# CagriCatik/RRT-MPC

Hardware: AMD Instinct MI355X
Metric: MPC QP solves/s (horizon=20, batch=4096) @1/2/4/8 GPU; rel-err vs OSQP (higher is better)
Workload: dtype f64

## Files before the change

### rrt-mpc_amd/csrc/mpcqp_common.h

```cpp
#pragma once
#include <hip/hip_runtime.h>

#include <chrono>
#include <cmath>
#include <cstdint>
#include <cstdio>
#include <cstring>
#include <functional>
#include <mutex>
#include <new>
#include <string>
#include <type_traits>
#include <utility>

#include "../../include/mpcqp.h"

namespace {

constexpr int kWave = 64;
constexpr double kPi = 3.141592653589793;
constexpr double kTwoPi = 6.283185307179586;
constexpr double kMinScaling = 1e-4;
constexpr double kMaxScaling = 1e4;
constexpr double kRhoMin = 1e-6;
// ... 79 lines not shown
  double off = row >= 1 ? t0 : 0.0;
  if (row >= 2) off = fmax(off, t1);
  if (row >= 3) off = fmax(off, t2);
  return fmax(v, off);
}
__device__ __forceinline__ double rscan_max(double v, int lane) {
  v = fmax(v, dpp<kRowShl1>(v));
  v = fmax(v, dpp<kRowShl2>(v));
  v = fmax(v, dpp<kRowShl4>(v));
  v = fmax(v, dpp<kRowShl8>(v));
  const double t1 = readlane(v, 16), t2 = readlane(v, 32), t3 = readlane(v, 48);
  const int row = lane >> 4;
  double off = row <= 2 ? t3 : 0.0;
  if (row <= 1) off = fmax(off, t2);
  if (row <= 0) off = fmax(off, t1);
  return fmax(v, off);
}
__device__ __forceinline__ double max_nc(double a, double b) {
  double r;
  asm("v_max_f64 %0, %1, %2" : "=v"(r) : "v"(a), "v"(b));
  return r;
}
__device__ __forceinline__ double min_nc(double a, double b) {
  double r;
  asm("v_min_f64 %0, %1, %2" : "=v"(r) : "v"(a), "v"(b));
  return r;
}
__device__ __forceinline__ double wave_sum(double v) { return readlane(scan_add(v, 0), 63); }
__device__ __forceinline__ void wave_sum2(double& a, double& b) {
  a += dpp<kRowShr1>(a);
  b += dpp<kRowShr1>(b);
  a += dpp<kRowShr2>(a);
  b += dpp<kRowShr2>(b);
  a += dpp<kRowShr4>(a);
  b += dpp<kRowShr4>(b);
  a += dpp<kRowShr8>(a);
  b += dpp<kRowShr8>(b);
  a += dpp_rows<kRowBcast15, 0xa>(a);
  b += dpp_rows<kRowBcast15, 0xa>(b);
  a += dpp_rows<kRowBcast31, 0xc>(a);
  b += dpp_rows<kRowBcast31, 0xc>(b);
  a = readlane(a, 63);
  b = readlane(b, 63);
}
__device__ __forceinline__ double wave_max(double v) {
  v = max_nc(v, dpp<kRowShr1>(v));
  v = max_nc(v, dpp<kRowShr2>(v));
  v = max_nc(v, dpp<kRowShr4>(v));
  v = max_nc(v, dpp<kRowShr8>(v));
  v = max_nc(v, dpp_rows<kRowBcast15, 0xa>(v));
  v = max_nc(v, dpp_rows<kRowBcast31, 0xc>(v));
  return readlane(v, 63);
}
#define MPCQP_MAX4_STEP(MOVE)                                             \
  {                                                                       \
    const double ta = MOVE(a), tb = MOVE(b), tc = MOVE(c), td = MOVE(d); \
    a = max_nc(a, ta);                                                    \
    b = max_nc(b, tb);                                                    \
    c = max_nc(c, tc);                                                    \
    d = max_nc(d, td);                                                    \
  }
__device__ __forceinline__ void half_max4_steps(double& a, double& b, double& c, double& d) {
  MPCQP_MAX4_STEP(dpp<kRowShr1>)
  MPCQP_MAX4_STEP(dpp<kRowShr2>)
  MPCQP_MAX4_STEP(dpp<kRowShr4>)
  MPCQP_MAX4_STEP(dpp<kRowShr8>)
  MPCQP_MAX4_STEP((dpp_rows<kRowBcast15, 0xa>))
}
__device__ __forceinline__ void wave_max4(double& a, double& b, double& c, double& d) {
  half_max4_steps(a, b, c, d);
  MPCQP_MAX4_STEP((dpp_rows<kRowBcast31, 0xc>))
  a = readlane(a, 63);
  b = readlane(b, 63);
  c = readlane(c, 63);
  d = readlane(d, 63);
}
#undef MPCQP_MAX4_STEP
__device__ __forceinline__ double shr2(double v) { return dpp<kWaveShr1>(dpp<kWaveShr1>(v)); }
__device__ __forceinline__ double shl2(double v) { return dpp<kWaveShl1>(dpp<kWaveShl1>(v)); }
__device__ __forceinline__ double shr4(double v) { return shr2(shr2(v)); }
__device__ __forceinline__ double shl4(double v) { return shl2(shl2(v)); }
__device__ __forceinline__ bool wave_any(bool b) { return __ballot(b) != 0ull; }

template <int NW>
__device__ __forceinline__ void bcast(double v, double w[4]) {
  const int lo = __double2loint(v), hi = __double2hiint(v);
  const auto l16 = __builtin_amdgcn_permlane16_swap(lo, lo, false, false);
  const auto h16 = __builtin_amdgcn_permlane16_swap(hi, hi, false, false);
  const auto la = __builtin_amdgcn_permlane32_swap(l16[0], l16[0], false, false);
  const auto ha = __builtin_amdgcn_permlane32_swap(h16[0], h16[0], false, false);
  w[0] = __hiloint2double(ha[0], la[0]);
  if constexpr (NW > 1) {
    const auto lb = __builtin_amdgcn_permlane32_swap(l16[1], l16[1], false, false);
    const auto hb = __builtin_amdgcn_permlane32_swap(h16[1], h16[1], false, false);
    w[1] = __hiloint2double(hb[0], lb[0]);
    if constexpr (NW > 3) w[3] = __hiloint2double(hb[1], lb[1]);
  }
  if constexpr (NW > 2) w[2] = __hiloint2double(ha[1], la[1]);
  if constexpr (NW == 1) asm volatile("s_nop 1" : "+v"(w[0]));
  if constexpr (NW == 2) asm volatile("s_nop 1" : "+v"(w[0]), "+v"(w[1]));
  if constexpr (NW == 3) asm volatile("s_nop 1" : "+v"(w[0]), "+v"(w[1]), "+v"(w[2]));
  if constexpr (NW == 4) asm volatile("s_nop 1" : "+v"(w[0]), "+v"(w[1]), "+v"(w[2]), "+v"(w[3]));
}
template <int NW>
__device__ __forceinline__ void bcast_rows01(double v, double w[4]) {
  static_assert(NW <= 2, "two 16-lane rows");
  if constexpr (NW == 1) {
    w[0] = v;
    asm volatile("s_nop 1" : "+v"(w[0]));
  } else {
    const int lo = __double2loint(v), hi = __double2hiint(v);
    const auto l16 = __builtin_amdgcn_permlane16_swap(lo, lo, false, false);
    const auto h16 = __builtin_amdgcn_permlane16_swap(hi, hi, false, false);
    w[0] = __hiloint2double(h16[0], l16[0]);
    w[1] = __hiloint2double(h16[1], l16[1]);
    asm volatile("s_nop 1" : "+v"(w[0]), "+v"(w[1]));
  }
}
template <int L>
__device__ __forceinline__ void fmac_bc(double& acc, double w, double m) {
  asm("v_fmac_f64_dpp %0, %1, %2 row_newbcast:%3 row_mask:0xf bank_mask:0xf" : "+v"(acc) : "v"(w), "v"(m), "i"(L));
}
template <bool Pair>
struct Lanes;

template <>
struct Lanes<false> {
  static constexpr int kLanes = kWave;
  template <int NW>
  __device__ __forceinline__ static void vbcast(double v, double w[4]) {
    if constexpr (NW <= 2)
      bcast_rows01<NW>(v, w);
    else
      bcast<NW>(v, w);
  }
  template <int K>
  __device__ __forceinline__ static double read(double v) { return readlane(v, K); }
  __device__ __forceinline__ static double readv(double v, int l) { return readlane(v, l); }
  __device__ __forceinline__ static int uniform(int l) { return __builtin_amdgcn_readfirstlane(l); }
  __device__ __forceinline__ static double sum(double v) { return wave_sum(v); }
  __device__ __forceinline__ static void sum2(double& a, double& b) { wave_sum2(a, b); }
  __device__ __forceinline__ static double max(double v) { return wave_max(v); }
  __device__ __forceinline__ static void max4(double& a, double& b, double& c, double& d) { wave_max4(a, b, c, d); }
  __device__ __forceinline__ static bool any(bool b) { return wave_any(b); }
  __device__ __forceinline__ static uint64_t ballot(bool b) { return __ballot(b); }
  __device__ __forceinline__ static double shr2(double v) { return ::shr2(v); }
  __device__ __forceinline__ static double shl2(double v) { return ::shl2(v); }
  __device__ __forceinline__ static double shr4(double v) { return ::shr4(v); }
  __device__ __forceinline__ static double shl4(double v) { return ::shl4(v); }
  __device__ __forceinline__ static double shr1(double v) { return dpp<kWaveShr1>(v); }
  __device__ __forceinline__ static double shl1(double v) { return dpp<kWaveShl1>(v); }
  __device__ __forceinline__ static double scan(double v, int lane) { return scan_add(v, lane); }
  __device__ __forceinline__ static double shfl(double v, int src) { return __shfl(v, src, kWave); }
};

template <int L>
__device__ __forceinline__ double row_bc(double v) {
  const int lo = __builtin_amdgcn_update_dpp(0, __double2loint(v), 0x150 + L, 0xf, 0xf, false);
  const int hi = __builtin_amdgcn_update_dpp(0, __double2hiint(v), 0x150 + L, 0xf, 0xf, false);
  return __hiloint2double(hi, lo);
}

template <>
struct Lanes<true> {
  static constexpr int kLanes = 32;
  __device__ __forceinline__ static int hl() { return (int)threadIdx.x & 31; }
  __device__ __forceinline__ static double pin(double v) {
    asm volatile("" : "+v"(v));
    return v;
  }
  template <int NW>
  __device__ __forceinline__ static void vbcast(double v, double w[4]) {
    static_assert(NW <= 2, "a half holds 32 lanes");
    bcast_rows01<2>(v, w);
  }
  template <int K>
  __device__ __forceinline__ static double read(double v) {
    double w[4];
    bcast_rows01<2>(v, w);
    return pin(row_bc<K % 16>(w[K / 16]));
  }
  __device__ __forceinline__ static double readv(double v, int l) { return pin(__shfl(v, l, 32)); }
  __device__ __forceinline__ static int uniform(int l) { return l; }
  __device__ __forceinline__ static double scan(double v, int lane) {
    (void)lane;
    v += dpp<kRowShr1>(v);
    v += dpp<kRowShr2>(v);
    v += dpp<kRowShr4>(v);
    v += dpp<kRowShr8>(v);
    v += dpp_rows<kRowBcast15, 0xa>(v);
    return pin(v);
  }
  __device__ __forceinline__ static double sum(double v) { return read<31>(scan(v, 0)); }
  __device__ __forceinline__ static void sum2(double& a, double& b) {
    a = sum(a);
    b = sum(b);
  }
  __device__ __forceinline__ static double max(double v) {
    v = max_nc(v, dpp<kRowShr1>(v));
    v = max_nc(v, dpp<kRowShr2>(v));
    v = max_nc(v, dpp<kRowShr4>(v));
    v = max_nc(v, dpp<kRowShr8>(v));
    v = max_nc(v, dpp_rows<kRowBcast15, 0xa>(v));
    return read<31>(v);
  }
  __device__ __forceinline__ static void max4(double& a, double& b, double& c, double& d) {
    half_max4_steps(a, b, c, d);
    a = read<31>(a);
    b = read<31>(b);
    c = read<31>(c);
    d = read<31>(d);
  }
  __device__ __forceinline__ static uint64_t ballot(bool b) {
    const uint64_t m = __ballot(b);
    return (threadIdx.x & 32) ? (m >> 32) : (m & 0xffffffffull);
  }
  __device__ __forceinline__ static bool any(bool b) { return ballot(b) != 0ull; }
  __device__ __forceinline__ static double shr2(double v) {
    const double d = pin(::shr2(v));
    return hl() >= 2 ? d : 0.0;
  }
  __device__ __forceinline__ static double shl2(double v) {
    const double d = pin(::shl2(v));
    return hl() < 30 ? d : 0.0;
  }
  __device__ __forceinline__ static double shr4(double v) { return shr2(shr2(v)); }
  __device__ __forceinline__ static double shl4(double v) { return shl2(shl2(v)); }
  __device__ __forceinline__ static double shr1(double v) {
    const double d = pin(dpp<kWaveShr1>(v));
    return hl() >= 1 ? d : 0.0;
  }
  __device__ __forceinline__ static double shl1(double v) {
    const double d = pin(dpp<kWaveShl1>(v));
    return hl() < 31 ? d : 0.0;
  }
  __device__ __forceinline__ static double shfl(double v, int src) { return pin(__shfl(v, src, 32)); }
};

template <int B, int E>
struct Unroll {
  template <class F>
  __device__ __forceinline__ static void run(F&& f) {
    if constexpr (B < E) {
      f(std::integral_constant<int, B>{});
      Unroll<B + 1, E>::run(f);
    }
  }
};

__device__ __forceinline__ void lds_sync() { __builtin_amdgcn_fence(__ATOMIC_SEQ_CST, "wavefront"); }

#ifdef MPCQP_PHASE_MARKS
#define MPCQP_MARK(name) asm volatile(";@phase " name)
#else
#define MPCQP_MARK(name)
#endif

// ... 240 lines not shown
```

### rrt-mpc_amd/csrc/mpcqp_solve.h

```cpp
#pragma once
#include "mpcqp_build.h"

namespace {
using mpcqp::Launch;

template <int N>
constexpr bool kPackedP = N >= 24;

template <int N, bool Packed = kPackedP<N>>
struct SolveSmem {
  static constexpr int n = 2 * N;
  static constexpr int kPS = n + 1;
  double pad0[4];
  double P[n * kPS];
  double pad1[4];
  double band[5][n];
};
template <int N>
struct SolveSmem<N, true> {
  static constexpr int n = 2 * N;
  static constexpr int kPS = 0;
  double P[kWave * (kWave + 1) / 2];
  double band[3][n];
};
__device__ __forceinline__ int tri_idx(int i, int j) { return i >= j ? (i * (i + 1)) / 2 + j : (j * (j + 1)) / 2 + i; }
template <int N>
__device__ __forceinline__ int interleaved(int p) {
  return p < N ? 2 * p : (p < 2 * N ? 2 * (p - N) + 1 : p);
}

constexpr int kColBytes = 2 * kWave * 8;
template <int N>
constexpr bool kModelKept =
    8 * ((int)sizeof(SolveSmem<N>) + kColBytes) + 64 * model_stride(N) <= 163840;

template <int N>
struct SetupSmem {
  static constexpr int n = 2 * N;
  double buf[kWave];
  double model[kModelKept<N> ? 1 : model_stride(N)];
  double pre[4][N + 1];
  double err[4][N + 1];
  double g[n];
  static constexpr int kBT = 2 * n - 1;
  double bt[4][kBT];
};

template <int N, bool Pair = false>
struct SolveLds {
  union {
    SetupSmem<N> setup;
    SolveSmem<N> solve;
  };
  double model[kModelKept<N> ? model_stride(N) : 1];
  double col[Pair ? 1 : 2 * kWave];
  __device__ double* model_ptr() { return kModelKept<N> ? model : setup.model; }
};

template <int N, bool Pair = false>
struct Ctx {
  using LN = Lanes<Pair>;
  static constexpr int n = 2 * N;
  int lane;
  bool act, even;
  double dt;
  double D, qv;
  double iE[3], lo[3], hi[3], wb[3];
  double c0, c10, c11, c20, c21, c22;
  double icscale;
  static constexpr int kPS = SolveSmem<N>::kPS;
  double* __restrict__ P;
  double* __restrict__ colb;
  const double* __restrict__ band;
  static constexpr int kNW = (n + 15) / 16;
  double r[n];
  int n_full, n_r1;

  __device__ __forceinline__ void init(int ln, double dt_, SolveSmem<N>& s) {
    lane = ln;
    band = &s.band[0][0];
    n_full = 0;
    n_r1 = 0;
    act = ln < n;
    even = ln < N;
    dt = dt_;
    P = s.P;
  }
// ... 249 lines not shown
    if constexpr (kRegBcast) vbcast(u, w);
    Unroll<0, n>::run([&](auto jc) {
      constexpr int j = decltype(jc)::value;
      fmac_bc<j % 16>(r[j], w[j / 16], m);
    });
    return true;
  }
  template <int I>
  __device__ __forceinline__ double r_or_zero() const {
    if constexpr (I >= 0) return r[I];
    else return 0.0;
  }
  template <int LO, int HI>
  __device__ __forceinline__ void pick3(int j, double& v0, double& v1, double& v2) const {
    if constexpr (HI - LO <= 2) {
      MPCQP_MARK("pol.pick_leaf");
      v0 = r[LO];
      v1 = r_or_zero<LO - 1>();
      v2 = r_or_zero<LO - 2>();
      if constexpr (HI - LO == 2) {
        const bool up = j == LO + 1;
        v0 = up ? r[LO + 1] : v0;
        v1 = up ? r[LO] : v1;
        v2 = up ? r_or_zero<LO - 1>() : v2;
      }
      asm volatile("" : "+v"(v0), "+v"(v1), "+v"(v2));
    } else {
      constexpr int M = (LO + HI) / 2;
      if (j < M) pick3<LO, M>(j, v0, v1, v2);
      else pick3<M, HI>(j, v0, v1, v2);
    }
  }
  __device__ __forceinline__ double inv_mul(double v) const {
    double w[4];
    if constexpr (!Pair && kNW <= 2)
      vbcast(act ? v : 0.0, w);
    else
      vbcast(v, w);
    double a[3] = {0.0, 0.0, 0.0};
    Unroll<0, n>::run([&](auto jc) {
      constexpr int j = decltype(jc)::value;
      fmac_bc<j % 16>(a[j % 3], w[j / 16], r[j]);
    });
    return -((a[0] + a[1]) + a[2]);
  }
};

struct BatchWin {
  static constexpr bool kFleet = false;
  __device__ __forceinline__ int lane() const { return threadIdx.x; }
};
struct FleetWin {
  static constexpr bool kFleet = true;
  const double* __restrict__ rows;
  int ln;
  int len, pidx;
  bool relax;
  double x[4], u[2];
  template <int N>
  __device__ __forceinline__ void row(int k, double& rx, double& ry, double& ryaw, double& rv) const {
    const double* r = rows + (size_t)min(pidx + k, len - 1) * 4;
    rx = r[0];
    ry = r[1];
    ryaw = r[2];
    rv = relax ? r[3] * 0.6 : r[3];
  }
  __device__ __forceinline__ double x0l(int lane) const {
    return lane == 0 ? x[0] : (lane == 1 ? x[1] : (lane == 2 ? x[2] : (lane == 3 ? x[3] : 0.0)));
  }
  __device__ __forceinline__ double upl(int lane) const { return lane == 4 ? u[0] : (lane == 5 ? u[1] : 0.0); }
  __device__ __forceinline__ int lane() const { return ln; }
  __device__ __forceinline__ double x0v(int i) const { return x[i]; }
  __device__ __forceinline__ double upv(int i) const { return u[i]; }
};

struct ServeWin {
  static constexpr bool kFleet = false;
  int ln;
  __device__ __forceinline__ int lane() const { return ln; }
};

struct ClassWin {
  static constexpr bool kFleet = false;
  __device__ __forceinline__ int lane() const { return threadIdx.x; }
};

template <int N, class Win, bool Pair = false>
__device__ __forceinline__ bool setup_qp(const mpcqp_params& p, int b, const double* __restrict__ model,
                                         const double* __restrict__ in_x0, const double* __restrict__ in_ref,
                                         const double* __restrict__ in_up, const Win& win, Ctx<N, Pair>& C,
                                         SolveLds<N, Pair>& lds, double* __restrict__ scratch, double* __restrict__ dbg) {
  using LN = Lanes<Pair>;
  constexpr int n = 2 * N;
  SetupSmem<N>& sm = lds.setup;
  (void)scratch;
  constexpr int S = model_stride(N);
  const int lane = win.lane();
  const bool act = lane < n;
  const bool even = act && lane < N;
  const int cc = lane >= N ? 1 : 0;
  const int kv = lane - cc * N;
  const double dt = p.dt;
  Stamps T, T2;
  T2.begin();
  T.begin();
  MPCQP_MARK("setup.k1");

  if constexpr (Win::kFleet) {
    double rx = 0.0, ry = 0.0, ryaw = 0.0, rv = 0.0;
    if (lane <= N) win.template row<N>(lane, rx, ry, ryaw, rv);
    build_qp<Pair>(p, lane, rx, ry, ryaw, rv, win.x0l(lane), win.upl(lane), lds.model_ptr());
  } else if (in_ref) {
    const double* rb = in_ref + (size_t)b * (N + 1) * 4;
    double rx = 0.0, ry = 0.0, ryaw = 0.0, rv = 0.0;
    if (lane <= N) {
      rx = rb[4 * lane + 0];
      ry = rb[4 * lane + 1];
      ryaw = rb[4 * lane + 2];
      rv = rb[4 * lane + 3];
    }
    const double x0l = lane < 4 ? in_x0[(size_t)b * 4 + lane] : 0.0;
    const double upl = (lane >= 4 && lane < 6 && in_up) ? in_up[(size_t)b * 2 + lane - 4] : 0.0;
    build_qp<Pair>(p, lane, rx, ry, ryaw, rv, x0l, upl, lds.model_ptr());
  } else {
    const double* mb = model + (size_t)b * S;
    double* md = lds.model_ptr();
    for (int i = lane; i < S; i += LN::kLanes) md[i] = mb[i];
  }
  __syncthreads();
  const double* mdl = lds.model_ptr();
  const double* al = mdl;
  const double* be = mdl + N;
  const double* ga = mdl + 2 * N;
  const double* et = mdl + 3 * N;
  const double* si = mdl + 4 * N;
  const double* c0 = mdl + 5 * N;
  const double* c1 = mdl + 6 * N;
  const double* rr = mdl + 7 * N;
  const double* x0 = mdl + 11 * N + 4;
  const double* up = mdl + 11 * N + 8;

  if constexpr (n < kWave) {
    constexpr int kBT = SetupSmem<N>::kBT;
    const double r00 = 0.5 * (p.r[0] + p.r[0]) / (dt * dt), r10 = 0.5 * (p.r[2] + p.r[1]) / dt;
    const double r11 = 0.5 * (p.r[3] + p.r[3]);
    for (int e = lane; e < 4 * kBT; e += LN::kLanes) {
      const int kind = e / kBT, d = e % kBT - (n - 1);
      double v = 0.0;
      if (kind == 0 || kind == 2) {
        if (d == 0) v = kind == 0 ? 2.0 * r00 : r00;
        if (d == -1 || (d == 1 && kind == 0)) v = -r00;
        if (d == N) v = r10;
        if (d == N + 1 && kind == 0) v = -r10;
      } else if (kind == 1) {
        if (d == 0) v = r11;
        if (d == -N) v = r10;
        if (d == -N - 1) v = -r10;
      }
      (&sm.bt[0][0])[e] = v;
    }
  }
  MPCQP_MARK("setup.prefix");
  if (lane < 4) {
    const bool fr = lane >= 2;
    const int q = lane & 1;
    const double* __restrict__ A = mdl + (q ? 2 * N : 0);
    const double* __restrict__ Bv = mdl + (q ? 3 * N : N);
    const double* __restrict__ Cc = mdl + (q ? 6 * N : 5 * N);
    const double* __restrict__ R = rr + 4 + q;
    const double h = fr ? x0[2] : 1.0, v0 = fr ? x0[3] : 0.0, one = fr ? 1.0 : 0.0;
    double acc = fr ? x0[q] : 0.0;
    double* __restrict__ out = fr ? sm.err[q] : sm.pre[2 * q];
    if (!fr) out[0] = 0.0;
    double a[N], c[N], r[N];
#pragma unroll
    for (int k = 0; k < N; ++k) {
      a[k] = A[k];
      c[k] = Cc[k];
      r[k] = R[4 * k];
    }
    const double b0 = Bv[0];
#pragma unroll
    for (int k = 0; k < N; ++k) {
      acc = acc + a[k] * h + (k == 0 ? b0 : 0.0) * (k == 0 ? v0 : 0.0) + one * c[k];
      out[k + 1] = acc - one * r[k];
    }
  }
  if (lane >= 1 && lane <= N) {
    sm.err[2][lane] = x0[2] - rr[4 * lane + 2];
    sm.err[3][lane] = 0.0 - rr[4 * lane + 3];
  }
  __syncthreads();
  T.end(0);
  T.begin();

  MPCQP_MARK("setup.condense");
  double Pc[n];
  if constexpr (n < kWave) {
#pragma unroll
    for (int i = 0; i < n; ++i) Pc[i] = 0.0;
    if (lane <= n) {
      const bool gcol = lane == n;
      const int j = kv;
      const double sj = gcol ? 1.0 : si[j];
      const double pa0 = gcol ? 0.0 : sm.pre[0][j + 1], pg0 = gcol ? 0.0 : sm.pre[2][j + 1];
      const double bj = (!gcol && j + 1 < N) ? be[j + 1] : 0.0, ej = (!gcol && j + 1 < N) ? et[j + 1] : 0.0;
      const bool st = gcol || cc == 1;
      const double k01 = st ? sj : 0.0, o0 = st ? pa0 : 0.0, o1 = st ? pg0 : 0.0;
      const double b0 = st ? 0.0 : bj, b1 = st ? 0.0 : ej;
      const double kg = gcol ? 1.0 : 0.0;
      const double c2v = (!gcol && cc == 1) ? sj : 0.0;
      const int t01 = gcol ? 0 : (cc == 1 ? j : j + 1);
      const int t2 = gcol ? 0 : j;
      const int t3 = (!gcol && cc == 0) ? j + 1 : -1;
      const double* X0 = gcol ? sm.err[0] : sm.pre[0];
      const double* X1 = gcol ? sm.err[1] : sm.pre[2];
      const double* X2 = gcol ? sm.err[2] : sm.pre[0];
      const double* X3 = gcol ? sm.err[3] : sm.pre[0];
      bool diag = true;
#pragma unroll
      for (int a = 0; a < 4; ++a)
#pragma unroll
        for (int b = 0; b < 4; ++b)
          if (a != b) diag = diag && p.q[4 * a + b] == 0.0 && p.q_terminal[4 * a + b] == 0.0;
      double mu0 = 0.0, mu1 = 0.0, mu2 = 0.0;
      auto recursion = [&](auto is_diag) {
        constexpr bool kDiag = decltype(is_diag)::value;
        if constexpr (kDiag)
          MPCQP_MARK("setup.condense");
        else
          MPCQP_MARK("setup.condense_full_q");
        double Q[4][4], QN[4][4];
#pragma unroll
        for (int a = 0; a < 4; ++a)
#pragma unroll
          for (int b = 0; b < 4; ++b) {
            Q[a][b] = 0.5 * (p.q[4 * a + b] + p.q[4 * b + a]);
            QN[a][b] = 0.5 * (p.q_terminal[4 * a + b] + p.q_terminal[4 * b + a]);
          }
#pragma unroll
        for (int m = N; m >= 1; --m) {
          double s0 = fma(k01, X0[m] - o0, b0);
          double s1 = fma(k01, X1[m] - o1, b1);
          s0 = m > t01 ? s0 : 0.0;
          s1 = m > t01 ? s1 : 0.0;
          const double s2 = fma(kg, X2[m], m > t2 ? c2v : 0.0);
          const double s3 = fma(kg, X3[m], m == t3 ? 1.0 : 0.0);
          const bool term = m == N;
          auto W = [&](int i, int k) -> double { return term ? QN[i][k] : Q[i][k]; };
          double w0, w1, w2, w3;
          if constexpr (kDiag) {
            w0 = W(0, 0) * s0;
            w1 = W(1, 1) * s1;
            w2 = W(2, 2) * s2;
            w3 = W(3, 3) * s3;
          } else {
            w0 = W(0, 0) * s0 + W(0, 1) * s1 + W(0, 2) * s2 + W(0, 3) * s3;
            w1 = W(1, 0) * s0 + W(1, 1) * s1 + W(1, 2) * s2 + W(1, 3) * s3;
            w2 = W(2, 0) * s0 + W(2, 1) * s1 + W(2, 2) * s2 + W(2, 3) * s3;
            w3 = W(3, 0) * s0 + W(3, 1) * s1 + W(3, 2) * s2 + W(3, 3) * s3;
          }
          double ha;
          if (m < N) {
            const double m0 = mu0, m1 = mu1;
            ha = w3 + (be[m] * m0 + et[m] * m1);
            mu0 = w0 + m0;
            mu1 = w1 + m1;
            mu2 = w2 + (mu2 + al[m] * m0 + ga[m] * m1);
          } else {
            ha = w3;
            mu0 = w0;
            mu1 = w1;
            mu2 = w2;
          }
          Pc[m - 1] = ha;
          Pc[N + m - 1] = si[m - 1] * mu2;
        }
      };
      if (diag)
        recursion(std::true_type{});
      else
        recursion(std::false_type{});
      MPCQP_MARK("setup.gcol");
      if (gcol)
#pragma unroll
        for (int i = 0; i < n; ++i) sm.g[i] = Pc[i];
      MPCQP_MARK("setup.band");
      if (gcol) {
        const double r00 = 0.5 * (p.r[0] + p.r[0]) / (dt * dt), r10 = 0.5 * (p.r[2] + p.r[1]) / dt;
        sm.g[0] += -x0[3] * r00;
        sm.g[N] += -x0[3] * r10;
      }
      const int kind = gcol ? 3 : (cc == 1 ? 1 : (lane + 1 < N ? 0 : 2));
      const double* tb = &sm.bt[kind][gcol ? 0 : n - 1 - lane];
#pragma unroll
      for (int i = 0; i < n; ++i) Pc[i] += tb[i];
    }
    __syncthreads();
    if (!act)
#pragma unroll
      for (int i = 0; i < n; ++i) Pc[i] = 0.0;
  } else {
#pragma unroll
    for (int i = 0; i < n; ++i) Pc[i] = 0.0;
    double Q[4][4], QN[4][4];
#pragma unroll
    for (int i = 0; i < 4; ++i)
#pragma unroll
      for (int j = 0; j < 4; ++j) {
        Q[i][j] = 0.5 * (p.q[4 * i + j] + p.q[4 * j + i]);
        QN[i][j] = 0.5 * (p.q_terminal[4 * i + j] + p.q_terminal[4 * j + i]);
      }
    const double r00 = 0.5 * (p.r[0] + p.r[0]) / (dt * dt), r10 = 0.5 * (p.r[2] + p.r[1]) / dt;
    const double r11 = 0.5 * (p.r[3] + p.r[3]);
#pragma nounroll
    for (int gpass = 0; gpass < 2; ++gpass) {
      const int j = kv;
      const bool gcol = gpass == 1;
      const double sj = gcol ? 0.0 : si[j];
      const double pa0 = gcol ? 0.0 : sm.pre[0][j + 1], pg0 = gcol ? 0.0 : sm.pre[2][j + 1];
      const double bj = (!gcol && j + 1 < N) ? be[j + 1] : 0.0, ej = (!gcol && j + 1 < N) ? et[j + 1] : 0.0;
      double mu0 = 0.0, mu1 = 0.0, mu2 = 0.0;
      Unroll<0, N>::run([&](auto mc) __attribute__((always_inline)) {
        constexpr int m = N - decltype(mc)::value;
        double s0, s1, s2, s3;
        if (gcol) {
          s0 = sm.err[0][m];
          s1 = sm.err[1][m];
          s2 = sm.err[2][m];
          s3 = sm.err[3][m];
// ... 74 lines not shown
  double qv = act ? 2.0 * sm.g[lane] : 0.0;
  double cmx[4] = {0.0, 0.0, 0.0, 0.0};
#pragma unroll
  for (int i = 0; i < n; ++i) {
    Pc[i] = 2.0 * Pc[i];
    cmx[i % 4] = fmax(cmx[i % 4], fabs(Pc[i]));
  }
  double cmax = fmax(fmax(cmx[0], cmx[1]), fmax(cmx[2], cmx[3]));
  double lo[3], hi[3], wt[3], E[3];
  const double idt = 1.0 / dt, v0 = x0[3];
  double k1[2], k2[3];
  k1[0] = act ? (even ? idt : 1.0) : 0.0;
  k1[1] = (even && kv >= 1) ? -idt : 0.0;
  k2[0] = act ? (even ? idt : 1.0) : 0.0;
  k2[1] = act ? (even ? (kv >= 1 ? -2.0 * idt : 0.0) : (kv >= 1 ? -1.0 : 0.0)) : 0.0;
  k2[2] = (even && kv >= 2) ? idt : 0.0;
  {
    const double ofa = lane == 0 ? v0 * idt : 0.0;
    const double ofr = (act && kv == 0) ? up[cc] + ofa : ((even && kv == 1) ? -v0 * idt : 0.0);
    lo[0] = even ? p.v_bounds[0] : 0.0;
    hi[0] = even ? p.v_bounds[1] : 0.0;
    wt[0] = even ? p.slack_velocity : 0.0;
    lo[1] = act ? p.u_bounds[2 * cc] + ofa : 0.0;
    hi[1] = act ? p.u_bounds[2 * cc + 1] + ofa : 0.0;
    wt[1] = act ? p.slack_input : 0.0;
    lo[2] = act ? p.du_bounds[2 * cc] + ofr : 0.0;
    hi[2] = act ? p.du_bounds[2 * cc + 1] + ofr : 0.0;
    wt[2] = act ? p.slack_rate : 0.0;
    E[0] = even ? 1.0 : 0.0;
    E[1] = act ? 1.0 : 0.0;
    E[2] = act ? 1.0 : 0.0;
  }
  double D = act ? 1.0 : 0.0;
  double cscale = 1.0;
  T.end(2);
  T.begin();

  auto rsqrt = [](double v) {
    double y = __builtin_amdgcn_rsq(v);
    y = y * fma(-0.5 * v, y * y, 1.5);
    return y * fma(-0.5 * v, y * y, 1.5);
  };
  double cpend = 1.0;
  MPCQP_MARK("setup.ruiz");
  for (int it = 0; it < p.scaling; ++it) {
    double ccol = fmax(fmax(E[0], E[1] * fabs(k1[0])), E[2] * fabs(k2[0]));
    ccol = fmax(ccol, LN::shl1(fmax(E[1] * fabs(k1[1]), E[2] * fabs(k2[1]))));
    ccol = fmax(ccol, LN::shl2(E[2] * fabs(k2[2])));
    ccol *= D;
    const double dl = act ? rsqrt(limit_scaling(fmax(cmax, ccol))) : 0.0;
    const double Dm1 = LN::shr1(D), Dm2 = LN::shr1(Dm1);
    const double r1 = fmax(fabs(k1[0]) * D, fabs(k1[1]) * Dm1);
    const double r2 = fmax(fmax(fabs(k2[0]) * D, fabs(k2[1]) * Dm1), fabs(k2[2]) * Dm2);
    const double el0 = even ? rsqrt(limit_scaling(E[0] * D)) : 0.0;
    const double el1 = act ? rsqrt(limit_scaling(E[1] * r1)) : 0.0;
    const double el2 = act ? rsqrt(limit_scaling(E[2] * r2)) : 0.0;
    lds_sync();
    sm.buf[lane] = dl;
    lds_sync();
    const double dlc = dl * cpend;
    double cmp[4] = {0.0, 0.0, 0.0, 0.0};
#pragma unroll
    for (int i = 0; i < n; ++i) {
      const double t = Pc[i] * (sm.buf[i] * dlc);
      Pc[i] = t;
      cmp[i % 4] = fmax(cmp[i % 4], fabs(t));
    }
    const double cm2 = fmax(fmax(cmp[0], cmp[1]), fmax(cmp[2], cmp[3]));
    D *= dl;
    qv *= dl;
    E[0] *= el0;
    E[1] *= el1;
    E[2] *= el2;
    const double cn = LN::sum(act ? cm2 : 0.0) / n;
    const double qn = limit_scaling(LN::max(fabs(qv)));
    const double ct = 1.0 / limit_scaling(fmax(cn, qn));
    cpend = ct;
    qv *= ct;
    cmax = cm2 * ct;
    cscale *= ct;
  }
#pragma unroll
  for (int i = 0; i < n; ++i) Pc[i] *= cpend;
  __syncthreads();
  T.end(3);
  T.begin();

  bool finite = isfinite(qv) && isfinite(cscale);
#pragma unroll 4
  for (int i = lane; i < 11 * N + 10; i += LN::kLanes) finite = finite && isfinite(mdl[i]);
  MPCQP_MARK("setup.write");
  lds_sync();
  if constexpr (kPackedP<N>) {
    double* Pb = lds.solve.P;
    if (act) {
#pragma unroll
      for (int i = 0; i < n; ++i)
        if (i >= lane) {
          Pb[(i * (i + 1)) / 2 + lane] = Pc[i];
          finite = finite && isfinite(Pc[i]);
        }
    }
    for (int e = (n * (n + 1)) / 2 + lane; e < kWave * (kWave + 1) / 2; e += kWave) Pb[e] = 0.0;
    lds_sync();
    if (act) {
      const double* rowp = Pb + (lane * (lane + 1)) / 2 + lane;
      lds.solve.band[0][lane] = lane >= 2 ? rowp[-2] : 0.0;
      lds.solve.band[1][lane] = lane >= 1 ? rowp[-1] : 0.0;
      lds.solve.band[2][lane] = rowp[0];
    }
  } else {
    constexpr int kPS = SolveSmem<N>::kPS;
    double* Pb = lds.solve.P;
    if (act) {
#pragma unroll
      for (int i = 0; i < n; ++i)
        if (i >= lane) {
          Pb[i * kPS + lane] = Pc[i];
          Pb[lane * kPS + i] = Pc[i];
          finite = finite && isfinite(Pc[i]);
        }
    } else if (lane == n) {
#pragma unroll
      for (int i = 0; i < n; ++i) Pb[i * kPS + n] = 0.0;
    }
    if (lane < 4) lds.solve.pad0[lane] = 0.0;
    else if (lane < 8) lds.solve.pad1[lane - 4] = 0.0;
    if constexpr (n >= 8) {
      lds_sync();
      if (act) {
        const double* rowp = Pb + lane * (kPS + 1);
#pragma unroll
        for (int d = 0; d < 5; ++d) lds.solve.band[d][lane] = rowp[d - 2];
      }
    }
  }
  double wb[3];
#pragma unroll
  for (int r = 0; r < 3; ++r) {
    lo[r] *= E[r];
    hi[r] *= E[r];
    wb[r] = E[r] > 0.0 ? cscale * wt[r] / (E[r] * E[r]) : 0.0;
    finite = finite && isfinite(lo[r]) && isfinite(hi[r]);
  }
  const bool bad_input = LN::any(!finite);
  C.init(lane, dt, lds.solve);
  C.colb = lds.col;
  C.qv = qv;
  C.D = D;
  C.icscale = 1.0 / cscale;
  {
    const double Dm1 = LN::shr1(D), Dm2 = LN::shr1(Dm1);
    C.c0 = E[0] * D;
    C.c10 = (E[1] * k1[0]) * D;
    C.c11 = (E[1] * k1[1]) * Dm1;
    C.c20 = (E[2] * k2[0]) * D;
    C.c21 = (E[2] * k2[1]) * Dm1;
    C.c22 = (E[2] * k2[2]) * Dm2;
  }
#pragma unroll
  for (int r = 0; r < 3; ++r) {
    C.iE[r] = E[r] > 0.0 ? 1.0 / E[r] : 0.0;
    C.lo[r] = lo[r];
    C.hi[r] = hi[r];
    C.wb[r] = wb[r];
  }
  __syncthreads();
  if (dbg) {
    const int il = interleaved<N>(lane);
    if (act)
      for (int i = 0; i < n; ++i)
        dbg[interleaved<N>(i) * n + il] =
            kPackedP<N> ? lds.solve.P[tri_idx(i, lane)] : lds.solve.P[i * SolveSmem<N>::kPS + lane];
    double* lf = dbg + state_lane_off(N);
    lf[kFq * kWave + il] = qv;
    lf[kFD * kWave + il] = D;
    lf[kFx * kWave + il] = 0.0;
#pragma unroll
    for (int r = 0; r < 3; ++r) {
      lf[(kFE0 + r) * kWave + il] = E[r];
      lf[(kFlo0 + r) * kWave + il] = lo[r];
      lf[(kFhi0 + r) * kWave + il] = hi[r];
      lf[(kFw0 + r) * kWave + il] = wb[r];
    }
    if (lane == 0) {
      double* sc = dbg + state_scal_off(N);
      sc[0] = cscale;
      sc[1] = bad_input ? -1.0 : 0.0;
      sc[2] = 0.0;
      sc[3] = 0.0;
    }
  }
  T.end(4);
  T2.end(0);
  MPCQP_MARK("ctl");
  T.flush(16);
  T2.flush(21);
  return bad_input;
}

template <int N, bool Pair = false>
__device__ __forceinline__ int polish_qp(Ctx<N, Pair>& C, double& x, const double zg[3], int max_it, int& pol_it,
                                         int& nfact, int& n_ls) {
  using LN = Lanes<Pair>;
  constexpr int n = 2 * N;
  const bool act = C.act;
  int result = 0;
  Stamps T;
  double zc[3];
  int cd[3];
  C.Cmul(x, zc);
  double Px = C.Pmul(x);
#pragma unroll
  for (int r = 0; r < 3; ++r) cd[r] = zg[r] > C.hi[r] ? 2 : (zg[r] < C.lo[r] ? 1 : 0);
  constexpr int kMaxRank1 = n / 2;
  double rwf[3] = {0.0, 0.0, 0.0};
  bool have_fact = false;
  for (int pass = 0; pass < max_it; ++pass) {
    MPCQP_MARK("pol.ctl");
// ... 949 lines not shown
  fleet_loop_body<N, false>(P + 2 * (size_t)c, f, steps, off, b, lane, sm, ls);
}

template <int N>
__global__ __launch_bounds__(kWave, kSolveWavesPerEU<N>) void k_fleet_loop_warm(const mpcqp_params* __restrict__ P,
                                                                              mpcqp_fleet f, int steps,
                                                                              int guess_passes,
                                                                              const int32_t* __restrict__ order) {
  __shared__ SolveLds<N> sm;
  __shared__ double ls[6];
  const int b = order ? order[blockIdx.x] : (int)blockIdx.x;
  const int lane = (int)threadIdx.x;
  if (b < 0 || b >= f.vehicles) return;
  const mpcqp::LoopTrigger off{0.0, 0, nullptr, nullptr};
  fleet_loop_body<N, false, true>(P, f, steps, off, b, lane, sm, ls, guess_passes);
}

template <int N>
__global__ __launch_bounds__(kWave, 1) void k_serve(mpcqp_params p, mpcqp::ServeLaunch L) {
  __shared__ SolveLds<N> sm;
  const int lane = threadIdx.x;
  uint32_t last = __builtin_amdgcn_readfirstlane(
      __hip_atomic_load(&L.box->done, __ATOMIC_RELAXED, __HIP_MEMORY_SCOPE_SYSTEM));
  for (;;) {
    const uint64_t t0 = __builtin_amdgcn_s_memrealtime();
    uint32_t req = last;
    while (req == last) {
      req = __builtin_amdgcn_readfirstlane(
          __hip_atomic_load(&L.box->req, __ATOMIC_RELAXED, __HIP_MEMORY_SCOPE_SYSTEM));
      if (req != last) break;
      if (__builtin_amdgcn_s_memrealtime() - t0 > L.idle_ticks) return;
      __builtin_amdgcn_s_sleep(1);
    }
    if (req == mpcqp::kServeStop) return;
    __builtin_amdgcn_fence(__ATOMIC_ACQUIRE, "");
    int ln = lane;
    asm volatile("" : "+v"(ln));
    const double* in = L.in;
    uint8_t* o = L.out;
    double Ul;
    solve_one<N>(p, 0, nullptr, in, in + 4, in + 4 + 4 * (N + 1), ServeWin{ln}, sm,
                 reinterpret_cast<double*>(o + L.off[0]), reinterpret_cast<double*>(o + L.off[1]),
                 reinterpret_cast<double*>(o + L.off[2]), reinterpret_cast<int32_t*>(o + L.off[3]),
                 reinterpret_cast<int32_t*>(o + L.off[4]), o + L.off[5], Ul);
    __builtin_amdgcn_fence(__ATOMIC_RELEASE, "");
    if (lane == 0) __hip_atomic_store(&L.box->done, req, __ATOMIC_RELAXED, __HIP_MEMORY_SCOPE_SYSTEM);
    last = req;
    __syncthreads();
  }
}

struct ServeGuessWin {
  static constexpr bool kFleet = false;
  int ln;
  __device__ __forceinline__ int lane() const { return ln; }
};

template <int N>
__global__ __launch_bounds__(kWave, 1) void k_serve_warm(mpcqp_params p, mpcqp::ServeWarmLaunch W) {
  __shared__ SolveLds<N> sm;
  const mpcqp::ServeLaunch& L = W.serve;
  const int lane = threadIdx.x;
  uint32_t last = __builtin_amdgcn_readfirstlane(
      __hip_atomic_load(&L.box->done, __ATOMIC_RELAXED, __HIP_MEMORY_SCOPE_SYSTEM));
  for (;;) {
    const uint64_t t0 = __builtin_amdgcn_s_memrealtime();
    uint32_t req = last;
    while (req == last) {
      req = __builtin_amdgcn_readfirstlane(
          __hip_atomic_load(&L.box->req, __ATOMIC_RELAXED, __HIP_MEMORY_SCOPE_SYSTEM));
      if (req != last) break;
      if (__builtin_amdgcn_s_memrealtime() - t0 > L.idle_ticks) return;
      __builtin_amdgcn_s_sleep(1);
    }
    if (req == mpcqp::kServeStop) return;
    __builtin_amdgcn_fence(__ATOMIC_ACQUIRE, "");
    int ln = lane;
    asm volatile("" : "+v"(ln));
    const int passes = __builtin_amdgcn_readfirstlane(
        __hip_atomic_load(W.passes, __ATOMIC_RELAXED, __HIP_MEMORY_SCOPE_SYSTEM));
    const double g = ln < 2 * N ? W.guess[ln] : 0.0;
    const double* in = L.in;
    uint8_t* o = L.out;
    double Ul;
    solve_one<N, ServeGuessWin, false, true>(p, 0, nullptr, in, in + 4, in + 4 + 4 * (N + 1), ServeGuessWin{ln}, sm,
                                        reinterpret_cast<double*>(o + L.off[0]), reinterpret_cast<double*>(o + L.off[1]),
                                        reinterpret_cast<double*>(o + L.off[2]), reinterpret_cast<int32_t*>(o + L.off[3]),
                                        reinterpret_cast<int32_t*>(o + L.off[4]), o + L.off[5], Ul, Guess<true>{g, passes});
    __builtin_amdgcn_fence(__ATOMIC_RELEASE, "");
    if (lane == 0) __hip_atomic_store(&L.box->done, req, __ATOMIC_RELAXED, __HIP_MEMORY_SCOPE_SYSTEM);
    last = req;
    __syncthreads();
  }
}

}

namespace mpcqp {
template <int N>
void launch_serve(hipStream_t s, const mpcqp_params& p, const ServeLaunch& L) {
  hipLaunchKernelGGL(k_serve<N>, dim3(1), dim3(kWave), 0, s, p, L);
}
template <int N>
void launch_serve_warm(hipStream_t s, const mpcqp_params& p, const ServeWarmLaunch& W) {
  hipLaunchKernelGGL(k_serve_warm<N>, dim3(1), dim3(kWave), 0, s, p, W);
}
// ... 57 lines not shown
```

Measured before the change: 24.33 million.

## Software-pipeline setup recursion loads, fuse sum/max reduction, and reorder setup phases

Restructures the per-solve setup phase. The backward Riccati-like recursion is software-pipelined, fetching operands for the next group of steps before computing the current group, with the group size depending on N and the window type. A fused wave sum+max reduction is added. Parameter-only work (diag check, bt table) is moved before build_qp for batch windows. Band extraction and the bad-input vote are deferred so the synchronisations overlap independent arithmetic. The model finiteness check now uses register-held loads. These change instruction scheduling and add register pressure, which may lower occupancy.

New measurement: 24.45 million (median of 6 runs). Within noise of the previous version (+0.5%).

```diff
diff --git a/rrt-mpc_amd/csrc/mpcqp_common.h b/rrt-mpc_amd/csrc/mpcqp_common.h
--- a/rrt-mpc_amd/csrc/mpcqp_common.h
+++ b/rrt-mpc_amd/csrc/mpcqp_common.h
@@ -155,6 +155,22 @@
   v = max_nc(v, dpp_rows<kRowBcast31, 0xc>(v));
   return readlane(v, 63);
 }
+__device__ __forceinline__ void wave_sum_max(double& s, double& m) {
+  s += dpp<kRowShr1>(s);
+  m = max_nc(m, dpp<kRowShr1>(m));
+  s += dpp<kRowShr2>(s);
+  m = max_nc(m, dpp<kRowShr2>(m));
+  s += dpp<kRowShr4>(s);
+  m = max_nc(m, dpp<kRowShr4>(m));
+  s += dpp<kRowShr8>(s);
+  m = max_nc(m, dpp<kRowShr8>(m));
+  s += dpp_rows<kRowBcast15, 0xa>(s);
+  m = max_nc(m, dpp_rows<kRowBcast15, 0xa>(m));
+  s += dpp_rows<kRowBcast31, 0xc>(s);
+  m = max_nc(m, dpp_rows<kRowBcast31, 0xc>(m));
+  s = readlane(s, 63);
+  m = readlane(m, 63);
+}
 #define MPCQP_MAX4_STEP(MOVE)                                             \
   {                                                                       \
     const double ta = MOVE(a), tb = MOVE(b), tc = MOVE(c), td = MOVE(d); \
@@ -244,6 +260,7 @@
   __device__ __forceinline__ static double sum(double v) { return wave_sum(v); }
   __device__ __forceinline__ static void sum2(double& a, double& b) { wave_sum2(a, b); }
   __device__ __forceinline__ static double max(double v) { return wave_max(v); }
+  __device__ __forceinline__ static void sum_max(double& s, double& m) { wave_sum_max(s, m); }
   __device__ __forceinline__ static void max4(double& a, double& b, double& c, double& d) { wave_max4(a, b, c, d); }
   __device__ __forceinline__ static bool any(bool b) { return wave_any(b); }
   __device__ __forceinline__ static uint64_t ballot(bool b) { return __ballot(b); }
@@ -306,6 +323,10 @@
     v = max_nc(v, dpp<kRowShr8>(v));
     v = max_nc(v, dpp_rows<kRowBcast15, 0xa>(v));
     return read<31>(v);
+  }
+  __device__ __forceinline__ static void sum_max(double& s, double& m) {
+    s = sum(s);
+    m = max(m);
   }
   __device__ __forceinline__ static void max4(double& a, double& b, double& c, double& d) {
     half_max4_steps(a, b, c, d);
diff --git a/rrt-mpc_amd/csrc/mpcqp_solve.h b/rrt-mpc_amd/csrc/mpcqp_solve.h
--- a/rrt-mpc_amd/csrc/mpcqp_solve.h
+++ b/rrt-mpc_amd/csrc/mpcqp_solve.h
@@ -33,6 +33,13 @@
 template <int N>
 constexpr bool kModelKept =
     8 * ((int)sizeof(SolveSmem<N>) + kColBytes) + 64 * model_stride(N) <= 163840;
+
+template <int N>
+constexpr int kCondGroup = N <= 5 ? 4 : (N <= 24 ? 2 : 1);
+template <class Win, class = void>
+struct ResidentWin : std::false_type {};
+template <class Win>
+struct ResidentWin<Win, std::void_t<decltype(Win::kResident)>> : std::bool_constant<Win::kResident> {};
 
 template <int N>
 struct SetupSmem {
@@ -388,6 +395,7 @@
 };
 struct FleetWin {
   static constexpr bool kFleet = true;
+  static constexpr bool kResident = true;
   const double* __restrict__ rows;
   int ln;
   int len, pidx;
@@ -412,6 +420,7 @@
 
 struct ServeWin {
   static constexpr bool kFleet = false;
+  static constexpr bool kResident = true;
   int ln;
   __device__ __forceinline__ int lane() const { return ln; }
 };
@@ -442,21 +451,59 @@
   T.begin();
   MPCQP_MARK("setup.k1");
 
+  double rx = 0.0, ry = 0.0, ryaw = 0.0, rv = 0.0, x0l = 0.0, upl = 0.0;
   if constexpr (Win::kFleet) {
-    double rx = 0.0, ry = 0.0, ryaw = 0.0, rv = 0.0;
     if (lane <= N) win.template row<N>(lane, rx, ry, ryaw, rv);
-    build_qp<Pair>(p, lane, rx, ry, ryaw, rv, win.x0l(lane), win.upl(lane), lds.model_ptr());
+    x0l = win.x0l(lane);
+    upl = win.upl(lane);
   } else if (in_ref) {
     const double* rb = in_ref + (size_t)b * (N + 1) * 4;
-    double rx = 0.0, ry = 0.0, ryaw = 0.0, rv = 0.0;
     if (lane <= N) {
       rx = rb[4 * lane + 0];
       ry = rb[4 * lane + 1];
       ryaw = rb[4 * lane + 2];
       rv = rb[4 * lane + 3];
     }
-    const double x0l = lane < 4 ? in_x0[(size_t)b * 4 + lane] : 0.0;
-    const double upl = (lane >= 4 && lane < 6 && in_up) ? in_up[(size_t)b * 2 + lane - 4] : 0.0;
+    x0l = lane < 4 ? in_x0[(size_t)b * 4 + lane] : 0.0;
+    upl = (lane >= 4 && lane < 6 && in_up) ? in_up[(size_t)b * 2 + lane - 4] : 0.0;
+  }
+
+  bool diag = true;
+  auto param_work = [&]() __attribute__((always_inline)) {
+    if constexpr (n < kWave) {
+#pragma unroll
+      for (int i = 0; i < 4; ++i)
+#pragma unroll
+        for (int j = 0; j < 4; ++j)
+          if (i != j) diag = diag & (p.q[4 * i + j] == 0.0) & (p.q_terminal[4 * i + j] == 0.0);
+    }
+
+    if constexpr (n < kWave) {
+      constexpr int kBT = SetupSmem<N>::kBT;
+      const double r00 = 0.5 * (p.r[0] + p.r[0]) / (dt * dt), r10 = 0.5 * (p.r[2] + p.r[1]) / dt;
+      const double r11 = 0.5 * (p.r[3] + p.r[3]);
+      for (int e = lane; e < 4 * kBT; e += LN::kLanes) {
+        const int kind = e / kBT, d = e % kBT - (n - 1);
+        double v = 0.0;
+        if (kind == 0 || kind == 2) {
+          if (d == 0) v = kind == 0 ? 2.0 * r00 : r00;
+          if (d == -1 || (d == 1 && kind == 0)) v = -r00;
+          if (d == N) v = r10;
+          if (d == N + 1 && kind == 0) v = -r10;
+        } else if (kind == 1) {
+          if (d == 0) v = r11;
+          if (d == -N) v = r10;
+          if (d == -N - 1) v = -r10;
+        }
+        (&sm.bt[0][0])[e] = v;
+      }
+    }
+  };
+  if constexpr (!ResidentWin<Win>::value) param_work();
+
+  if constexpr (Win::kFleet) {
+    build_qp<Pair>(p, lane, rx, ry, ryaw, rv, x0l, upl, lds.model_ptr());
+  } else if (in_ref) {
     build_qp<Pair>(p, lane, rx, ry, ryaw, rv, x0l, upl, lds.model_ptr());
   } else {
     const double* mb = model + (size_t)b * S;
@@ -464,6 +511,7 @@
     for (int i = lane; i < S; i += LN::kLanes) md[i] = mb[i];
   }
   __syncthreads();
+  if constexpr (ResidentWin<Win>::value) param_work();
   const double* mdl = lds.model_ptr();
   const double* al = mdl;
   const double* be = mdl + N;
@@ -476,26 +524,6 @@
   const double* x0 = mdl + 11 * N + 4;
   const double* up = mdl + 11 * N + 8;
 
-  if constexpr (n < kWave) {
-    constexpr int kBT = SetupSmem<N>::kBT;
-    const double r00 = 0.5 * (p.r[0] + p.r[0]) / (dt * dt), r10 = 0.5 * (p.r[2] + p.r[1]) / dt;
-    const double r11 = 0.5 * (p.r[3] + p.r[3]);
-    for (int e = lane; e < 4 * kBT; e += LN::kLanes) {
-      const int kind = e / kBT, d = e % kBT - (n - 1);
-      double v = 0.0;
-      if (kind == 0 || kind == 2) {
-        if (d == 0) v = kind == 0 ? 2.0 * r00 : r00;
-        if (d == -1 || (d == 1 && kind == 0)) v = -r00;
-        if (d == N) v = r10;
-        if (d == N + 1 && kind == 0) v = -r10;
-      } else if (kind == 1) {
-        if (d == 0) v = r11;
-        if (d == -N) v = r10;
-        if (d == -N - 1) v = -r10;
-      }
-      (&sm.bt[0][0])[e] = v;
-    }
-  }
   MPCQP_MARK("setup.prefix");
   if (lane < 4) {
     const bool fr = lane >= 2;
@@ -553,12 +581,6 @@
       const double* X1 = gcol ? sm.err[1] : sm.pre[2];
       const double* X2 = gcol ? sm.err[2] : sm.pre[0];
       const double* X3 = gcol ? sm.err[3] : sm.pre[0];
-      bool diag = true;
-#pragma unroll
-      for (int a = 0; a < 4; ++a)
-#pragma unroll
-        for (int b = 0; b < 4; ++b)
-          if (a != b) diag = diag && p.q[4 * a + b] == 0.0 && p.q_terminal[4 * a + b] == 0.0;
       double mu0 = 0.0, mu1 = 0.0, mu2 = 0.0;
       auto recursion = [&](auto is_diag) {
         constexpr bool kDiag = decltype(is_diag)::value;
@@ -574,14 +596,32 @@
             Q[a][b] = 0.5 * (p.q[4 * a + b] + p.q[4 * b + a]);
             QN[a][b] = 0.5 * (p.q_terminal[4 * a + b] + p.q_terminal[4 * b + a]);
           }
-#pragma unroll
-        for (int m = N; m >= 1; --m) {
-          double s0 = fma(k01, X0[m] - o0, b0);
-          double s1 = fma(k01, X1[m] - o1, b1);
+        struct StepOps {
+          double x0, x1, x2, x3, be, et, al, ga, si;
+        };
+        constexpr int kCG = ResidentWin<Win>::value ? 1 : kCondGroup<N>;
+        auto fetch = [&](auto mc, StepOps& o) __attribute__((always_inline)) {
+          constexpr int m = decltype(mc)::value;
+          o.x0 = X0[m];
+          o.x1 = X1[m];
+          o.x2 = X2[m];
+          o.x3 = X3[m];
+          if constexpr (m < N) {
+            o.be = be[m];
+            o.et = et[m];
+            o.al = al[m];
+            o.ga = ga[m];
+          }
+          o.si = si[m - 1];
+        };
+        auto step = [&](auto mc, const StepOps& o) __attribute__((always_inline)) {
+          constexpr int m = decltype(mc)::value;
+          double s0 = fma(k01, o.x0 - o0, b0);
+          double s1 = fma(k01, o.x1 - o1, b1);
           s0 = m > t01 ? s0 : 0.0;
           s1 = m > t01 ? s1 : 0.0;
-          const double s2 = fma(kg, X2[m], m > t2 ? c2v : 0.0);
-          const double s3 = fma(kg, X3[m], m == t3 ? 1.0 : 0.0);
+          const double s2 = fma(kg, o.x2, m > t2 ? c2v : 0.0);
+          const double s3 = fma(kg, o.x3, m == t3 ? 1.0 : 0.0);
           const bool term = m == N;
           auto W = [&](int i, int k) -> double { return term ? QN[i][k] : Q[i][k]; };
           double w0, w1, w2, w3;
@@ -597,12 +637,12 @@
             w3 = W(3, 0) * s0 + W(3, 1) * s1 + W(3, 2) * s2 + W(3, 3) * s3;
           }
           double ha;
-          if (m < N) {
+          if constexpr (m < N) {
             const double m0 = mu0, m1 = mu1;
-            ha = w3 + (be[m] * m0 + et[m] * m1);
+            ha = w3 + (o.be * m0 + o.et * m1);
             mu0 = w0 + m0;
             mu1 = w1 + m1;
-            mu2 = w2 + (mu2 + al[m] * m0 + ga[m] * m1);
+            mu2 = w2 + (mu2 + o.al * m0 + o.ga * m1);
           } else {
             ha = w3;
             mu0 = w0;
@@ -610,8 +650,29 @@
             mu2 = w2;
           }
           Pc[m - 1] = ha;
-          Pc[N + m - 1] = si[m - 1] * mu2;
-        }
+          Pc[N + m - 1] = o.si * mu2;
+        };
+        StepOps cur[kCG], nxt[kCG];
+        Unroll<0, kCG>::run([&](auto kc) __attribute__((always_inline)) {
+          constexpr int k = decltype(kc)::value;
+          if constexpr (k < N) fetch(std::integral_constant<int, N - k>{}, cur[k]);
+        });
+        Unroll<0, (N + kCG - 1) / kCG>::run([&](auto gc) __attribute__((always_inline)) {
+          constexpr int g = decltype(gc)::value;
+          Unroll<0, kCG>::run([&](auto kc) __attribute__((always_inline)) {
+            constexpr int k = decltype(kc)::value, s = (g + 1) * kCG + k;
+            if constexpr (s < N) fetch(std::integral_constant<int, N - s>{}, nxt[k]);
+          });
+          __builtin_amdgcn_sched_barrier(0);
+          Unroll<0, kCG>::run([&](auto kc) __attribute__((always_inline)) {
+            constexpr int k = decltype(kc)::value, s = g * kCG + k;
+            if constexpr (s < N) step(std::integral_constant<int, N - s>{}, cur[k]);
+          });
+          Unroll<0, kCG>::run([&](auto kc) __attribute__((always_inline)) {
+            constexpr int k = decltype(kc)::value;
+            if constexpr ((g + 1) * kCG + k < N) cur[k] = nxt[k];
+          });
+        });
       };
       if (diag)
         recursion(std::true_type{});
@@ -792,12 +853,12 @@
     const double Dm1 = LN::shr1(D), Dm2 = LN::shr1(Dm1);
     const double r1 = fmax(fabs(k1[0]) * D, fabs(k1[1]) * Dm1);
     const double r2 = fmax(fmax(fabs(k2[0]) * D, fabs(k2[1]) * Dm1), fabs(k2[2]) * Dm2);
+    lds_sync();
+    sm.buf[lane] = dl;
+    lds_sync();
     const double el0 = even ? rsqrt(limit_scaling(E[0] * D)) : 0.0;
     const double el1 = act ? rsqrt(limit_scaling(E[1] * r1)) : 0.0;
     const double el2 = act ? rsqrt(limit_scaling(E[2] * r2)) : 0.0;
-    lds_sync();
-    sm.buf[lane] = dl;
-    lds_sync();
     const double dlc = dl * cpend;
     double cmp[4] = {0.0, 0.0, 0.0, 0.0};
 #pragma unroll
@@ -812,50 +873,48 @@
     E[0] *= el0;
     E[1] *= el1;
     E[2] *= el2;
-    const double cn = LN::sum(act ? cm2 : 0.0) / n;
-    const double qn = limit_scaling(LN::max(fabs(qv)));
+    double csum = act ? cm2 : 0.0, qmax = fabs(qv);
+    LN::sum_max(csum, qmax);
+    const double cn = csum / n;
+    const double qn = limit_scaling(qmax);
     const double ct = 1.0 / limit_scaling(fmax(cn, qn));
     cpend = ct;
     qv *= ct;
     cmax = cm2 * ct;
     cscale *= ct;
   }
+  constexpr int kMW = 11 * N + 10, kMR = (kMW + LN::kLanes - 1) / LN::kLanes;
+  double mw[kMR];
+#pragma unroll
+  for (int k = 0; k < kMR; ++k) mw[k] = mdl[min(lane + k * LN::kLanes, kMW - 1)];
 #pragma unroll
   for (int i = 0; i < n; ++i) Pc[i] *= cpend;
   __syncthreads();
   T.end(3);
   T.begin();
 
-  bool finite = isfinite(qv) && isfinite(cscale);
-#pragma unroll 4
-  for (int i = lane; i < 11 * N + 10; i += LN::kLanes) finite = finite && isfinite(mdl[i]);
+  bool finite = isfinite(qv) & isfinite(cscale);
+#pragma unroll
+  for (int k = 0; k < kMR; ++k) finite = finite & isfinite(mw[k]);
   MPCQP_MARK("setup.write");
   lds_sync();
+  double* Pb = lds.solve.P;
   if constexpr (kPackedP<N>) {
-    double* Pb = lds.solve.P;
     if (act) {
 #pragma unroll
       for (int i = 0; i < n; ++i)
-        if (i >= lane) {
+        if (__builtin_expect(i >= lane, 1)) {
           Pb[(i * (i + 1)) / 2 + lane] = Pc[i];
           finite = finite && isfinite(Pc[i]);
         }
     }
     for (int e = (n * (n + 1)) / 2 + lane; e < kWave * (kWave + 1) / 2; e += kWave) Pb[e] = 0.0;
-    lds_sync();
-    if (act) {
-      const double* rowp = Pb + (lane * (lane + 1)) / 2 + lane;
-      lds.solve.band[0][lane] = lane >= 2 ? rowp[-2] : 0.0;
-      lds.solve.band[1][lane] = lane >= 1 ? rowp[-1] : 0.0;
-      lds.solve.band[2][lane] = rowp[0];
-    }
   } else {
     constexpr int kPS = SolveSmem<N>::kPS;
-    double* Pb = lds.solve.P;
     if (act) {
 #pragma unroll
       for (int i = 0; i < n; ++i)
-        if (i >= lane) {
+        if (__builtin_expect(i >= lane, 1)) {
           Pb[i * kPS + lane] = Pc[i];
           Pb[lane * kPS + i] = Pc[i];
           finite = finite && isfinite(Pc[i]);
@@ -866,24 +925,16 @@
     }
     if (lane < 4) lds.solve.pad0[lane] = 0.0;
     else if (lane < 8) lds.solve.pad1[lane - 4] = 0.0;
-    if constexpr (n >= 8) {
-      lds_sync();
-      if (act) {
-        const double* rowp = Pb + lane * (kPS + 1);
-#pragma unroll
-        for (int d = 0; d < 5; ++d) lds.solve.band[d][lane] = rowp[d - 2];
-      }
-    }
   }
   double wb[3];
 #pragma unroll
   for (int r = 0; r < 3; ++r) {
     lo[r] *= E[r];
     hi[r] *= E[r];
-    wb[r] = E[r] > 0.0 ? cscale * wt[r] / (E[r] * E[r]) : 0.0;
-    finite = finite && isfinite(lo[r]) && isfinite(hi[r]);
-  }
-  const bool bad_input = LN::any(!finite);
+    const double wq = cscale * wt[r] / (E[r] * E[r]);
+    wb[r] = E[r] > 0.0 ? wq : 0.0;
+    finite = finite & isfinite(lo[r]) & isfinite(hi[r]);
+  }
   C.init(lane, dt, lds.solve);
   C.colb = lds.col;
   C.qv = qv;
@@ -900,11 +951,34 @@
   }
 #pragma unroll
   for (int r = 0; r < 3; ++r) {
-    C.iE[r] = E[r] > 0.0 ? 1.0 / E[r] : 0.0;
+    const double ie = 1.0 / E[r];
+    C.iE[r] = E[r] > 0.0 ? ie : 0.0;
     C.lo[r] = lo[r];
     C.hi[r] = hi[r];
     C.wb[r] = wb[r];
   }
+  asm volatile("" ::"v"(wb[0]), "v"(wb[1]), "v"(wb[2]), "v"(C.iE[0]), "v"(C.iE[1]), "v"(C.iE[2]), "v"(C.icscale));
+  if constexpr (kPackedP<N>) {
+    lds_sync();
+    if (act) {
+      const double* rowp = Pb + (lane * (lane + 1)) / 2 + lane;
+      const double b0 = lane >= 2 ? rowp[-2] : 0.0, b1 = lane >= 1 ? rowp[-1] : 0.0, b2 = rowp[0];
+      lds.solve.band[0][lane] = b0;
+      lds.solve.band[1][lane] = b1;
+      lds.solve.band[2][lane] = b2;
+    }
+  } else if constexpr (n >= 8) {
+    lds_sync();
+    if (act) {
+      const double* rowp = Pb + lane * (SolveSmem<N>::kPS + 1);
+      double bs[5];
+#pragma unroll
+      for (int d = 0; d < 5; ++d) bs[d] = rowp[d - 2];
+#pragma unroll
+      for (int d = 0; d < 5; ++d) lds.solve.band[d][lane] = bs[d];
+    }
+  }
+  const bool bad_input = LN::any(!finite);
   __syncthreads();
   if (dbg) {
     const int il = interleaved<N>(lane);
@@ -1960,6 +2034,7 @@
 
 struct ServeGuessWin {
   static constexpr bool kFleet = false;
+  static constexpr bool kResident = true;
   int ln;
   __device__ __forceinline__ int lane() const { return ln; }
 };
```
